# jafarinia/snuffy

Hardware: AMD Instinct MI355X
Metric: slides/sec (higher is better)
Workload: dtype f32; 1 GPU; cfgB: MILNet eval forward, 1 bag/step/rank, N=32768 patches D=768 h=6 Lambda=200 (K=200) depth=1 relu mlp x4; parallelism=bag-parallel x1, bags_resident_per_rank=8, launch=hip graph replay, rccl_ranks=0

## Files before the change

### snuffy_amd/csrc/gemm.hip

```cpp
#include <stdlib.h>

#include "mfma.h"
#include "philox.h"

namespace {

struct GemmParams {
    const unsigned short* a;
    const unsigned short* w;
    const float* bias;
    void* c;
    int64_t lda, ldw, ldc;
    int m, n, k;
    int act;
    int tiles_m, tiles_n;
    unsigned long long* trace;
    const float* resid = nullptr;
    int64_t ldr = 0;
    unsigned int* split_cnt = nullptr;
    float* split_slab = nullptr;
    int split_cap = 0, split_rcap = 0;
    const unsigned short* gate = nullptr;
    int64_t ldg = 0;
    const float* colsum = nullptr;
    const float* rowstats = nullptr;
    unsigned short* c2 = nullptr;
    int64_t ldc2 = 0;
    float* stats_part = nullptr;
    int slots = 0;
    snf::DropoutState drop = {0u, 0u, 0u, 0u, 0u, 1.f};
};
constexpr int HL_SPLIT_MIN_STEPS = 8;
constexpr int HL_SPLIT_MAX = 4;

constexpr int BM = 256, BKS = 32;
constexpr int NBUF = 4, AHEAD = 2;
constexpr int ROWB = BKS * 2;
constexpr int A_BYTES = BM * ROWB;

__device__ __forceinline__ unsigned int cvt_pk_bf16(float lo, float hi) {
    return __builtin_bit_cast(unsigned int, __builtin_convertvector(f32x2{lo, hi}, bf16x2));
}

__device__ __forceinline__ float erf_as(float x) {
    const float ax = fabsf(x);
    const float t = __builtin_amdgcn_rcpf(fmaf(0.3275911f, ax, 1.0f));
    float p = fmaf(1.061405429f, t, -1.453152027f);
    p = fmaf(p, t, 1.421413741f);
    p = fmaf(p, t, -0.284496736f);
    p = fmaf(p, t, 0.254829592f);
    const float e = __builtin_amdgcn_exp2f(-ax * ax * 1.44269504088896340736f);
    return copysignf(fmaf(-p * t, e, 1.0f), x);
}

template <int ACT>
__device__ __forceinline__ float activate(float v) {
    if constexpr (ACT == SNF_ACT_RELU) return fmaxf(v, 0.f);
    if constexpr (ACT == SNF_ACT_GELU) return 0.5f * v * (1.0f + erf_as(v * 0.70710678118654752440f));
    if constexpr (ACT == SNF_ACT_LEAKYRELU) return v > 0.f ? v : 0.01f * v;
    if constexpr (ACT == SNF_ACT_SELU) {
        const float al = 1.6732632423543772848170429916717f, sc = 1.0507009873554804934193349852946f;
        return sc * (v > 0.f ? v : al * (__builtin_amdgcn_exp2f(v * 1.44269504088896340736f) - 1.0f));
    }
    return v;
}

template <int NI, int ACT, int OUT, int EPI = 0, int MI = 8, bool DROP = false>
__global__ __launch_bounds__(512, 2) void gemm_bf16_kernel(GemmParams P) {
    static_assert(!DROP || (ACT == SNF_ACT_RELU && OUT == 0 && EPI == 0), "gemm_bf16: dropout goes with the ReLU -> bf16 form");
    static_assert(MI == 8 || (MI == 4 && NI == 4 && EPI != 1), "gemm_bf16: wave tiles are 128 x 16 NI or 64 x 64");
    constexpr int WC = MI == 8 ? 4 : 2;
    constexpr int RW = 16 * MI;
    static_assert(EPI == 0 || (EPI == 1 ? (NI == 4 && OUT == 0) : ((NI == 4 || NI == 2) && OUT == 1 && ACT == SNF_ACT_NONE)),
                  "gemm_bf16: the LayerNorm-fold epilogue is 256-wide, the residual epilogue 256- or 128-wide");
    constexpr int BN = WC * 16 * NI;
    constexpr int W_BYTES = BN * ROWB;
    constexpr int STEP_BYTES = A_BYTES + W_BYTES;
    constexpr int WP = BN / 128;
    constexpr int GL = 2 + WP;
    constexpr int NC = 4 * NI;
    constexpr bool OUT_F32 = OUT == 1;
    constexpr int NST = EPI == 2 ? NC / 4 + NC / 8 + 1 : (OUT == 1 || OUT == 3) ? NC / 4 : OUT == 2 ? 3 * NC / 8 : NC / 8;
    static_assert((AHEAD - 1) * GL + MI * NST <= 63, "gemm_bf16: counted waits are 6-bit");
    constexpr bool LINE_STORES = OUT == 0 && NI == 4 && EPI != 2 && ACT != SNF_ACT_GELU && ACT != SNF_ACT_SELU;
    extern __shared__ __attribute__((aligned(16))) unsigned char smem[];

// ... 342 lines not shown
        const bool has_next = next < t_hi;
        const Src nxt = tile_src(has_next ? next : tile);
        const bool full = (tile / P.tiles_n + 1) * BM <= P.m && (tile % P.tiles_n + 1) * BN <= P.n;
        for (int s = 0; s < ns; ++s) {
            if constexpr (EPI == 2)
                if (s == 0) preload_x(tile);
            read_frags(rb);
            if (s == ns - 1) load_bias(tile);
            const bool in_tile = s + AHEAD < ns;
            const int exist = has_next ? AHEAD : (ns - 1 - s < AHEAD ? ns - 1 - s : AHEAD);
            if (in_tile)
                stage(cur, s + AHEAD, sb);
            else if (has_next)
                stage(nxt, s + AHEAD - ns, sb);
            if (exist == AHEAD) {
                if (after_epilogue)
                    wait_vmcnt<(AHEAD - 1) * GL + MI * NST>();
                else
                    wait_vmcnt<(AHEAD - 1) * GL>();
            } else if (AHEAD == 3 && exist == 2) {
                wait_vmcnt<GL>();
            } else {
                wait_vmcnt<0>();
            }
            after_epilogue = false;
            rb = rb == NBUF - 1 ? 0 : rb + 1;
            sb = sb == NBUF - 1 ? 0 : sb + 1;
            barrier();
            if (s == 0)
                mma(std::true_type{});
            else
                mma(std::false_type{});
            barrier();
        }
        bias_landed();
#ifdef SNF_GEMM_NOSTORE
        if (false) {
#else
        if (full) {
#endif
            epilogue(tile, std::true_type{});
            after_epilogue = true;
        } else {
            epilogue(tile, std::false_type{});
            wait_vmcnt<0>();
        }
        if (!has_next) break;
        tile = next;
        cur = nxt;
    }
    if (wid < 4) __builtin_amdgcn_s_barrier();
}

template <int ACT, int OUT, bool SPLIT = false, bool GATE = false, bool DROP = false>
__global__ __launch_bounds__(512, 2) void gemm_hl_kernel(GemmParams P) {
    static_assert(!GATE || (OUT == 3 && ACT == SNF_ACT_NONE && !SPLIT), "gemm_hl: the gated form writes an hl image, no activation, no split");
    static_assert(!DROP || (!GATE && (OUT == 1 || OUT == 3)), "gemm_hl: dropout goes with the fp32 and the hl-image outputs");
    constexpr int NI = 4, BN = 256;
    constexpr int ROWL = 128;
    constexpr int IMG = BM * ROWL;
    constexpr int STEP_BYTES = 2 * IMG;
    constexpr int NC = 4 * NI;
    constexpr bool LINE_STORES = (OUT == 1 || OUT == 3) && ACT != SNF_ACT_GELU && ACT != SNF_ACT_SELU;
    extern __shared__ __attribute__((aligned(16))) unsigned char smem[];

    const int lane = threadIdx.x & 63;
    const int wid = __builtin_amdgcn_readfirstlane(threadIdx.x >> 6);
    const int wr = wid >> 2, wc = wid & 3;
    const int ns_all = P.k / BKS;
    unsigned char* const scr = smem + 2 * STEP_BYTES + wid * 4096;

    const int ntiles = P.tiles_m * P.tiles_n;
    const int xcd = blockIdx.x & 7, wg_in_xcd = blockIdx.x >> 3, wgs_per_xcd = gridDim.x >> 3;
    if constexpr (!SPLIT) {
        if (P.split_cap >= 2 && blockIdx.x == 0) {
            for (int i = threadIdx.x; i < 8 * P.split_rcap; i += 512) P.split_cnt[i] = 0u;
            asm volatile("s_waitcnt vmcnt(0)" ::: "memory");
        }
    }
    int t_lo, t_hi;
    {
        const int q = ntiles >> 3, r = ntiles & 7;
        t_lo = xcd < r ? xcd * (q + 1) : r * (q + 1) + (xcd - r) * q;
        t_hi = t_lo + q + (xcd < r ? 1 : 0);
    }
    int sp_part = 0, sp_parts = 1, sp_slot = 0, sp_tile = -1;
    if (P.split_cap >= 2) {
        const int q_x = t_hi - t_lo, full_rounds = q_x / wgs_per_xcd, r = q_x - full_rounds * wgs_per_xcd;
        int sn = r > 0 ? wgs_per_xcd / r : 0;
        if (sn > P.split_cap) sn = P.split_cap;
        if (sn > ns_all / HL_SPLIT_MIN_STEPS) sn = ns_all / HL_SPLIT_MIN_STEPS;
        if (sn >= 2 && r <= P.split_rcap) {
            if constexpr (SPLIT) {
                if (wg_in_xcd < r * sn) {
                    const int jr = wg_in_xcd % r;
                    sp_tile = t_lo + full_rounds * wgs_per_xcd + jr;
                    sp_part = wg_in_xcd / r, sp_parts = sn, sp_slot = xcd * P.split_rcap + jr;
                }
            } else {
                t_hi = t_lo + full_rounds * wgs_per_xcd;
            }
        }
    }
    int tile = t_lo + wg_in_xcd;
    if constexpr (SPLIT) {
        tile = __builtin_amdgcn_readfirstlane(sp_tile);
        sp_part = __builtin_amdgcn_readfirstlane(sp_part), sp_parts = __builtin_amdgcn_readfirstlane(sp_parts);
        sp_slot = __builtin_amdgcn_readfirstlane(sp_slot);
        if (tile < 0) return;
        t_hi = tile + 1;
        asm volatile("" : "+s"(t_hi));
    } else {
        if (tile >= t_hi) return;
    }
    const int s_begin = SPLIT ? __builtin_amdgcn_readfirstlane(sp_part * ns_all / sp_parts) : 0;
    const int ns = SPLIT ? __builtin_amdgcn_readfirstlane((sp_part + 1) * ns_all / sp_parts) - s_begin : ns_all;
    const unsigned short* const a_base = P.a + (SPLIT ? s_begin * 64 : 0);
    const unsigned short* const w_base = P.w + (SPLIT ? s_begin * 64 : 0);

    struct Src {
        int a[4], w[4];
    };
    auto tile_src_mn = [&](int tm, int tn) __attribute__((always_inline)) -> Src {
        Src s;
        int ln = lane;
        asm volatile("" : "+v"(ln));
        const int c = ln & 7;
#pragma unroll
        for (int j = 0; j < 4; ++j) {
            const int row = (4 * wid + j) * 8 + (ln >> 3);
            int grow = tm * BM + row;
            if (grow > P.m - 1) grow = P.m - 1;
            s.a[j] = grow * (int)P.lda + ((c ^ ((row >> 1) & 7)) << 3);
            int wrow = tn * BN + row;
            if (wrow > P.n - 1) wrow = P.n - 1;
            s.w[j] = wrow * (int)P.ldw + ((c ^ (((row >> 1) & 1) | (((row >> 3) & 3) << 1))) << 3);
        }
        return s;
    };
    auto tile_src = [&](int tl) __attribute__((always_inline)) -> Src {
        const int tm = tl / P.tiles_n;
        return tile_src_mn(tm, tl - tm * P.tiles_n);
    };
    auto stage = [&](const Src& s, int kstep, int buf) __attribute__((always_inline)) {
#ifdef X3_NOSTAGE
        return;
#endif
        unsigned char* base = smem + buf * STEP_BYTES;
#pragma unroll
        for (int j = 0; j < 4; ++j) {
            __builtin_amdgcn_global_load_lds((glb_void*)(a_base + s.a[j] + kstep * 64), (lds_void*)(base + (4 * wid + j) * 1024), 16, 0, 0);
            __builtin_amdgcn_global_load_lds((glb_void*)(w_base + s.w[j] + kstep * 64), (lds_void*)(base + IMG + (4 * wid + j) * 1024), 16, 0, 0);
        }
    };

    const int fi = lane & 15, fg = lane >> 4;
    const int fa = (fi >> 1) & 7, fw = ((fi >> 1) & 1) | ((fi >> 2) << 1);
    const int xoff_h = (128 * wr + fi) * ROWL + ((fg ^ fa) << 4), xoff_l = (128 * wr + fi) * ROWL + (((4 + fg) ^ fa) << 4);
    const int wrow0 = IMG + (64 * wc + 8 * (fi >> 2) + (fi & 3)) * ROWL;
    const int woff_h = wrow0 + ((fg ^ fw) << 4), woff_l = wrow0 + (((4 + fg) ^ fw) << 4);

    f32x4 acc[8][NI];
    bf16x8 xf[8], wh[NI], wl[NI];
    f32x4 bv4[NC / 4];

    auto frag = [&](const unsigned char* p) __attribute__((always_inline)) -> bf16x8 {
#ifdef X3_NOREAD
        u32x4 z = {1u, 2u, 3u, (unsigned)lane};
        asm volatile("" : "+v"(z));
        return __builtin_bit_cast(bf16x8, z);
#endif
// ... 81 lines not shown
                    } else if (ok) {
                        *reinterpret_cast<f32x4*>(dst) = f32x4{v[0], v[1], v[2], v[3]};
                        *reinterpret_cast<f32x4*>(dst + 4) = f32x4{v[4], v[5], v[6], v[7]};
                    }
                } else {
                    const u32x4 pk = {cvt_pk_bf16(v[0], v[1]), cvt_pk_bf16(v[2], v[3]), cvt_pk_bf16(v[4], v[5]), cvt_pk_bf16(v[6], v[7])};
                    if constexpr (OUT == 0) {
                        unsigned short* dst = reinterpret_cast<unsigned short*>(P.c) + (int64_t)row * P.ldc + col;
                        if (ok) *reinterpret_cast<u32x4*>(dst) = pk;
                    } else {
                        float lo[8];
#pragma unroll
                        for (int e = 0; e < 8; ++e)
                            lo[e] = v[e] - __uint_as_float((e & 1) ? (pk[e >> 1] & 0xffff0000u) : (pk[e >> 1] << 16));
                        const u32x4 pl = {cvt_pk_bf16(lo[0], lo[1]), cvt_pk_bf16(lo[2], lo[3]), cvt_pk_bf16(lo[4], lo[5]), cvt_pk_bf16(lo[6], lo[7])};
                        unsigned short* dst = reinterpret_cast<unsigned short*>(P.c) + (int64_t)row * P.ldc + 64 * (col >> 5) + (col & 31);
                        if constexpr (LINE_STORES) {
                            *reinterpret_cast<u32x4*>(scr + fio * 256 + (((8 * h + fgo) ^ fio) << 4)) = pk;
                            *reinterpret_cast<u32x4*>(scr + fio * 256 + (((8 * h + 4 + fgo) ^ fio) << 4)) = pl;
                        } else if (ok) {
                            *reinterpret_cast<u32x4*>(dst) = pk;
                            *reinterpret_cast<u32x4*>(dst + 32) = pl;
                        }
                    }
                }
            }
            if constexpr (LINE_STORES) {
                const int lr = lane_o >> 4, lc = lane_o & 15;
                unsigned char* const crow = reinterpret_cast<unsigned char*>(P.c) +
                                            (OUT == 1 ? 4 * (int64_t)(tn * BN + 64 * wc) : 2 * 2 * (int64_t)(tn * BN + 64 * wc));
                const int64_t pitch = (OUT == 1 ? 4 : 2) * P.ldc;
#pragma unroll
                for (int jj = 0; jj < 4; ++jj) {
                    const int r = lr + 4 * jj;
                    const u32x4 val = *reinterpret_cast<const u32x4*>(scr + r * 256 + ((lc ^ r) << 4));
                    const int orow = tm * BM + 128 * wr + 16 * mi + r;
                    const int ocol = tn * BN + 64 * wc + (OUT == 1 ? 4 * lc : 32 * (lc >> 3) + 8 * (lc & 3));
#ifdef X3_NOSTORE
                    const bool ok2 = val[0] == 0x12345678u && orow < 0;
#else
                    const bool ok2 = FULL || (orow < P.m && ocol + (OUT == 1 ? 4 : 8) <= P.n);
#endif
                    if (ok2) *reinterpret_cast<u32x4*>(crow + orow * pitch + 16 * lc) = val;
                }
            }
        }
    };

    Src cur = tile_src(tile);
    stage(cur, 0, 0);
    int buf = 0;
    bool after_epilogue = false;
    while (true) {
        const int next = tile + wgs_per_xcd;
        const bool has_next = next < t_hi;
        const bool full = (tile / P.tiles_n + 1) * BM <= P.m && (tile % P.tiles_n + 1) * BN <= P.n;
        for (int s = 0; s < ns; ++s) {
            if (!(s == 0 && after_epilogue)) wait_vmcnt<0>();
            after_epilogue = false;
            __builtin_amdgcn_sched_barrier(0);
            __builtin_amdgcn_s_barrier();
            __builtin_amdgcn_sched_barrier(0);
            const unsigned char* base = smem + buf * STEP_BYTES;
#pragma unroll
            for (int ni = 0; ni < NI; ++ni) wh[ni] = frag(base + woff_h + (4 * (ni & 1) + 32 * (ni >> 1)) * ROWL);
#pragma unroll
            for (int mi = 0; mi < 8; ++mi) xf[mi] = frag(base + xoff_h + mi * 16 * ROWL);
#pragma unroll
            for (int ni = 0; ni < NI; ++ni) wl[ni] = frag(base + woff_l + (4 * (ni & 1) + 32 * (ni >> 1)) * ROWL);
            __builtin_amdgcn_sched_barrier(0);
            if (s + 1 < ns) {
                stage(cur, s + 1, buf ^ 1);
            } else if (has_next) {
                cur = tile_src(next);
                stage(cur, 0, buf ^ 1);
            }
            __builtin_amdgcn_sched_barrier(0);
            __builtin_amdgcn_s_setprio(1);
            if (s == 0) {
#pragma unroll
                for (int mi = 0; mi < 8; ++mi)
#pragma unroll
                    for (int ni = 0; ni < NI; ++ni) acc[mi][ni] = X3_MFMA(wh[ni], xf[mi], (f32x4{0.f, 0.f, 0.f, 0.f}));
            } else {
#pragma unroll
                for (int mi = 0; mi < 8; ++mi)
#pragma unroll
                    for (int ni = 0; ni < NI; ++ni) acc[mi][ni] = X3_MFMA(wh[ni], xf[mi], acc[mi][ni]);
            }
#pragma unroll
            for (int mi = 0; mi < 8; ++mi) {
#pragma unroll
                for (int ni = 0; ni < NI; ++ni) acc[mi][ni] = X3_MFMA(wl[ni], xf[mi], acc[mi][ni]);
                __builtin_amdgcn_sched_barrier(0);
                xf[mi] = frag(base + xoff_l + mi * 16 * ROWL);
                __builtin_amdgcn_sched_barrier(0);
            }
#pragma unroll
            for (int mi = 0; mi < 8; ++mi)
#pragma unroll
                for (int ni = 0; ni < NI; ++ni) acc[mi][ni] = X3_MFMA(wh[ni], xf[mi], acc[mi][ni]);
            __builtin_amdgcn_s_setprio(0);
            buf ^= 1;
        }
        if constexpr (SPLIT) {
            volatile unsigned int& s_ticket = *reinterpret_cast<volatile unsigned int*>(smem);
            float* slab0 = P.split_slab + (size_t)sp_slot * P.split_cap * (size_t)(BM * BN);
            unsigned tix = threadIdx.x;
            asm volatile("" : "+v"(tix));
            f32x4* mine = reinterpret_cast<f32x4*>(slab0 + (size_t)sp_part * (BM * BN)) + tix;
            wait_vmcnt<0>();
#pragma unroll
            for (int mi = 0; mi < 8; ++mi)
#pragma unroll
                for (int ni = 0; ni < NI; ++ni) mine[(mi * NI + ni) * 512] = acc[mi][ni];
            wait_vmcnt<0>();
            __syncthreads();
            if (tix == 0) {
                __builtin_amdgcn_fence(__ATOMIC_RELEASE, "agent");
                asm volatile("s_waitcnt vmcnt(0)" ::: "memory");
                s_ticket = __hip_atomic_fetch_add(P.split_cnt + sp_slot, 1u, __ATOMIC_RELAXED, __HIP_MEMORY_SCOPE_AGENT);
            }
            __syncthreads();
            if (s_ticket != (unsigned)(sp_parts - 1)) return;
            __syncthreads();
            if (tix == 0) {
                __builtin_amdgcn_fence(__ATOMIC_ACQUIRE, "agent");
                __hip_atomic_store(P.split_cnt + sp_slot, 0u, __ATOMIC_RELAXED, __HIP_MEMORY_SCOPE_AGENT);
            }
            __syncthreads();
#pragma unroll
            for (int mi = 0; mi < 8; ++mi)
#pragma unroll
                for (int ni = 0; ni < NI; ++ni) {
                    f32x4 sum = {0.f, 0.f, 0.f, 0.f};
                    for (int pp = 0; pp < sp_parts; ++pp) {
                        f32x4 v = acc[mi][ni];
                        if (pp != sp_part) v = reinterpret_cast<const f32x4*>(slab0 + (size_t)pp * (BM * BN))[(mi * NI + ni) * 512 + tix];
                        sum = pp == 0 ? v : sum + v;
                    }
                    acc[mi][ni] = sum;
                }
        }
        load_bias(tile);
        wait_vmcnt<0>();
        bias_landed();
        if (full)
            epilogue(tile, std::true_type{});
        else
            epilogue(tile, std::false_type{});
        after_epilogue = true;
        if (!has_next) break;
        tile = next;
    }
}

template <int ACT, int OUT, bool DROP = false>
int launch_hl(const GemmParams& P, hipStream_t s) {
    constexpr int lds = 2 * 2 * BM * 128 + (((OUT == 1 || OUT == 3) && ACT != SNF_ACT_GELU && ACT != SNF_ACT_SELU) ? 8 * 4096 : 0);
    auto kern = [] {
        if constexpr (DROP) return gemm_hl_kernel<ACT, OUT, false, false, true>;
        else return gemm_hl_kernel<ACT, OUT>;
    }();
    static thread_local unsigned long long attr_set_mask = 0;
    if (int rc = snf::lds_opt_in(reinterpret_cast<const void*>(kern), lds, &attr_set_mask, "gemm_hl")) return rc;
    const int ntiles = P.tiles_m * P.tiles_n;
    int grid = snf::cu_count() & ~7;
    if (grid < 8) grid = 8;
    {
        static const int dbg_grid = getenv("SNF_GEMM_HL_GRID") ? atoi(getenv("SNF_GEMM_HL_GRID")) & ~7 : 0;
        if (dbg_grid >= 8 && dbg_grid < grid && P.split_cap < 2) grid = dbg_grid;
    }
    const int per_xcd = (ntiles + 7) / 8;
    if (per_xcd * 8 < grid) grid = per_xcd * 8;
    hipLaunchKernelGGL(kern, dim3(grid), dim3(512), lds, s, P);
    int rc = snf::check_launch("gemm_hl_kernel");
    if (rc || P.split_cap < 2) return rc;
    auto kern2 = [] {
        if constexpr (DROP) return gemm_hl_kernel<ACT, OUT, true, false, true>;
        else return gemm_hl_kernel<ACT, OUT, true>;
    }();
    static thread_local unsigned long long attr_set2_mask = 0;
    if (int rc = snf::lds_opt_in(reinterpret_cast<const void*>(kern2), lds, &attr_set2_mask, "gemm_hl")) return rc;
    hipLaunchKernelGGL(kern2, dim3(grid), dim3(512), lds, s, P);
    return snf::check_launch("gemm_hl_kernel<split>");
}

int launch_hl_gated(const GemmParams& P, hipStream_t s) {
    constexpr int lds = 2 * 2 * BM * 128 + 8 * 4096;
    auto kern = gemm_hl_kernel<SNF_ACT_NONE, 3, false, true>;
    static thread_local unsigned long long attr_set_mask = 0;
    if (int rc = snf::lds_opt_in(reinterpret_cast<const void*>(kern), lds, &attr_set_mask, "gemm_hl")) return rc;
    const int ntiles = P.tiles_m * P.tiles_n;
    int grid = snf::cu_count() & ~7;
    if (grid < 8) grid = 8;
    const int per_xcd = (ntiles + 7) / 8;
    if (per_xcd * 8 < grid) grid = per_xcd * 8;
    hipLaunchKernelGGL(kern, dim3(grid), dim3(512), lds, s, P);
    return snf::check_launch("gemm_hl_kernel<gated>");
}

template <int OUT>
int launch_hl_act(const GemmParams& P, hipStream_t s) {
    switch (P.act) {
        case SNF_ACT_RELU: return launch_hl<SNF_ACT_RELU, OUT>(P, s);
        case SNF_ACT_GELU: return launch_hl<SNF_ACT_GELU, OUT>(P, s);
        case SNF_ACT_LEAKYRELU: return launch_hl<SNF_ACT_LEAKYRELU, OUT>(P, s);
        case SNF_ACT_SELU: return launch_hl<SNF_ACT_SELU, OUT>(P, s);
        default: return launch_hl<SNF_ACT_NONE, OUT>(P, s);
    }
}

template <int NI, int ACT, int OUT, int EPI = 0, int MI = 8, bool DROP = false>
int launch(const GemmParams& P, hipStream_t s) {
    constexpr int lds = NBUF * (A_BYTES + (MI == 8 ? 64 : 32) * NI * ROWB) +
                        ((EPI == 2 || (OUT == 0 && NI == 4 && ACT != SNF_ACT_GELU && ACT != SNF_ACT_SELU)) ? 8 * 4096 : 0);
    auto kern = [] {
        if constexpr (DROP) return gemm_bf16_kernel<NI, ACT, OUT, EPI, MI, true>;
        else return gemm_bf16_kernel<NI, ACT, OUT, EPI, MI>;
    }();
    static thread_local unsigned long long attr_set_mask = 0;
    if (int rc = snf::lds_opt_in(reinterpret_cast<const void*>(kern), lds, &attr_set_mask, "gemm_bf16")) return rc;
    const int ntiles = P.tiles_m * P.tiles_n;
    int grid = snf::cu_count() & ~7;
    if (grid < 8) grid = 8;
    const int per_xcd = (ntiles + 7) / 8;
    if (per_xcd * 8 < grid) grid = per_xcd * 8;
    hipLaunchKernelGGL(kern, dim3(grid), dim3(512), lds, s, P);
    return snf::check_launch("gemm_bf16_kernel");
}

#ifndef SNF_GEMM_128_MI4
#define SNF_GEMM_128_MI4 1
#endif
template <int NI, int ACT, int OUT, int EPI = 0, bool DROP = false>
int launch_tile(const GemmParams& P, hipStream_t s) {
    if constexpr (NI == 2 && SNF_GEMM_128_MI4)
        return launch<4, ACT, OUT, EPI, 4, DROP>(P, s);
// ... 260 lines not shown
    P.c = c;
    P.lda = lda, P.ldw = ldw, P.ldc = ldc;
    P.m = (int)m, P.n = n, P.k = k, P.act = act;
    P.tiles_m = (int)((m + BM - 1) / BM);
    P.tiles_n = (n + 255) / 256;
    P.trace = nullptr;
    return P;
}
}

extern "C" int snf_gemm_bf16_lnfold(const void* a, int64_t lda, const void* w, int64_t ldw, const float* colsum, const float* bias,
                                    const float* rowstats, int64_t m, int n, int k, int act, void* c, int64_t ldc, snf_stream_t stream) {
    SNF_REQUIRE(a && w && c && colsum && bias && rowstats, "snf_gemm_bf16_lnfold: null pointer");
    SNF_REQUIRE(m >= 1 && n >= 1 && k >= 1, "snf_gemm_bf16_lnfold: bad shape m=%lld n=%d k=%d", (long long)m, n, k);
    SNF_REQUIRE(act == SNF_ACT_NONE || act == SNF_ACT_GELU, "snf_gemm_bf16_lnfold: activation %d not built (none, gelu)", act);
    int rc = epi_domain("snf_gemm_bf16_lnfold", a, lda, w, ldw, m, n, k);
    if (rc) return rc;
    SNF_REQUIRE(ldc >= n && ldc % 8 == 0 && reinterpret_cast<uintptr_t>(c) % 16 == 0 && reinterpret_cast<uintptr_t>(colsum) % 16 == 0 &&
                    reinterpret_cast<uintptr_t>(bias) % 16 == 0 && reinterpret_cast<uintptr_t>(rowstats) % 8 == 0,
                "snf_gemm_bf16_lnfold: output / vector alignment");
    GemmParams P = epi_params(a, lda, w, ldw, bias, m, n, k, act, c, ldc);
    P.colsum = colsum, P.rowstats = rowstats;
    hipStream_t s = snf::as_stream(stream);
    return act == SNF_ACT_GELU ? launch<4, SNF_ACT_GELU, 0, 1>(P, s) : launch<4, SNF_ACT_NONE, 0, 1>(P, s);
}

extern "C" int snf_gemm_bf16_resid(const void* a, int64_t lda, const void* w, int64_t ldw, const float* bias, int64_t m, int n, int k,
                                   float* x, int64_t ldx, void* x_bf16, int64_t ldxb, float* stats_part, snf_stream_t stream) {
    SNF_REQUIRE(a && w && x && x_bf16 && stats_part && bias, "snf_gemm_bf16_resid: null pointer");
    SNF_REQUIRE(m >= 1 && n >= 1 && k >= 1, "snf_gemm_bf16_resid: bad shape m=%lld n=%d k=%d", (long long)m, n, k);
    int rc = epi_domain("snf_gemm_bf16_resid", a, lda, w, ldw, m, n, k);
    if (rc) return rc;
    SNF_REQUIRE(ldx >= n && ldx % 4 == 0 && ldxb >= n && ldxb % 8 == 0 && reinterpret_cast<uintptr_t>(x) % 16 == 0 &&
                    reinterpret_cast<uintptr_t>(x_bf16) % 16 == 0 && reinterpret_cast<uintptr_t>(bias) % 16 == 0 &&
                    reinterpret_cast<uintptr_t>(stats_part) % 16 == 0 && m * ldx < 0x7fffffffll,
                "snf_gemm_bf16_resid: output / vector alignment");
    GemmParams P = epi_params(a, lda, w, ldw, bias, m, n, k, SNF_ACT_NONE, x, ldx);
    P.c2 = reinterpret_cast<unsigned short*>(x_bf16), P.ldc2 = ldxb;
    P.stats_part = stats_part, P.slots = n / 32;
    const int rem = n % 256;
    if (rem >= 1 && rem <= 128) {
        P.tiles_n = (n + 127) / 128;
        return launch_tile<2, SNF_ACT_NONE, 1, 2>(P, snf::as_stream(stream));
    }
    return launch<4, SNF_ACT_NONE, 1, 2>(P, snf::as_stream(stream));
}

extern "C" int snf_gemm_hl_bf16(const void* a_hl, int64_t lda, const void* w_hl, int64_t ldw, const float* bias, int64_t m, int n,
                                int k, int act, void* c, int64_t ldc, int out_dtype, snf_stream_t stream) {
    return snf_gemm_hl_resid_bf16(a_hl, lda, w_hl, ldw, bias, nullptr, 0, m, n, k, act, c, ldc, out_dtype, stream);
}

namespace {
struct HlSplit {
    int cap, rcap;
};
HlSplit hl_split_geometry(int64_t m, int n, int k) {
    HlSplit g = {0, 0};
    if (m < 1 || n < 1 || k < BKS) return g;
    const int64_t ntiles64 = ((m + BM - 1) / BM) * ((n + 255) / 256);
    if (ntiles64 > 0x7fffffff) return g;
    const int ntiles = (int)ntiles64, ns = k / BKS;
    int grid = snf::cu_count() & ~7;
    if (grid < 8) grid = 8;
    const int per_xcd = (ntiles + 7) / 8;
    if (per_xcd * 8 < grid) grid = per_xcd * 8;
    const int w = grid >> 3;
    if (ntiles > 2 * grid) return g;
    for (int x = 0; x < 8; ++x) {
        const int q = ntiles / 8 + (x < (ntiles & 7) ? 1 : 0), r = q % w;
        if (r == 0) continue;
        int sn = w / r;
        if (sn > HL_SPLIT_MAX) sn = HL_SPLIT_MAX;
        if (sn > ns / HL_SPLIT_MIN_STEPS) sn = ns / HL_SPLIT_MIN_STEPS;
        if (sn < 2) continue;
        if (sn > g.cap) g.cap = sn;
        if (r > g.rcap) g.rcap = r;
    }
    if (g.cap < 2) g.cap = g.rcap = 0;
    return g;
}
constexpr size_t HL_TICKET_BYTES = 4096;
}

extern "C" size_t snf_gemm_hl_ws_bytes(int64_t m, int n, int k) {
    const HlSplit g = hl_split_geometry(m, n, k);
    if (g.cap < 2 || 8 * g.rcap * sizeof(unsigned int) > HL_TICKET_BYTES) return 0;
    return HL_TICKET_BYTES + (size_t)8 * g.rcap * g.cap * (size_t)(BM * 256) * sizeof(float);
}

extern "C" int snf_gemm_hl_resid_bf16(const void* a_hl, int64_t lda, const void* w_hl, int64_t ldw, const float* bias,
                                      const float* resid, int64_t ldr, int64_t m, int n, int k, int act, void* c, int64_t ldc,
                                      int out_dtype, snf_stream_t stream) {
    return snf_gemm_hl_ws_bf16(a_hl, lda, w_hl, ldw, bias, resid, ldr, m, n, k, act, c, ldc, out_dtype, nullptr, 0, stream);
}

namespace {
int gemm_hl_ws_impl(const void* a_hl, int64_t lda, const void* w_hl, int64_t ldw, const float* bias, const float* resid, int64_t ldr,
                    int64_t m, int n, int k, int act, void* c, int64_t ldc, int out_dtype, const snf::DropoutState* drop, void* workspace,
                    size_t workspace_bytes, snf_stream_t stream) {
    SNF_REQUIRE(a_hl && w_hl && c, "snf_gemm_hl_bf16: null pointer");
    SNF_REQUIRE(m >= 1 && n >= 1 && k >= 1, "snf_gemm_hl_bf16: bad shape m=%lld n=%d k=%d", (long long)m, n, k);
    SNF_REQUIRE(act >= SNF_ACT_RELU && act <= SNF_ACT_NONE, "snf_gemm_hl_bf16: bad activation code %d", act);
    SNF_REQUIRE(out_dtype == SNF_DT_F32 || out_dtype == SNF_DT_BF16 || out_dtype == SNF_DT_BF16_HL,
                "snf_gemm_hl_bf16: bad output dtype %d", out_dtype);
    const bool hl_out = out_dtype == SNF_DT_BF16_HL;
    SNF_REQUIRE(!resid || (out_dtype == SNF_DT_F32 && ldr >= n && ldr % 4 == 0 && reinterpret_cast<uintptr_t>(resid) % 16 == 0),
                "snf_gemm_hl_bf16: a residual needs an fp32 output and 16-byte aligned rows (ldr=%lld)", (long long)ldr);
    if (k % BKS || k < BKS || n % 8 || (hl_out && n % 32) || lda % 8 || ldw % 8 || ldc % (out_dtype == SNF_DT_F32 ? 4 : 8) ||
        lda < 2 * (int64_t)k || ldw < 2 * (int64_t)k || ldc < (hl_out ? 2 * (int64_t)n : n) ||
        (reinterpret_cast<uintptr_t>(a_hl) | reinterpret_cast<uintptr_t>(w_hl) | reinterpret_cast<uintptr_t>(c)) % 16 ||
        (bias && reinterpret_cast<uintptr_t>(bias) % 16) || m * lda >= 0x7fffffffll || (int64_t)n * ldw >= 0x7fffffffll) {
        snf::set_error("snf_gemm_hl_bf16: shape m=%lld n=%d k=%d (lda %lld ldw %lld ldc %lld) outside the kernel's domain "
                       "(k %% 32, n %% 8 (%% 32 for an hl output), images of 2 k columns, 16-byte aligned rows, 31-bit element offsets)",
                       (long long)m, n, k, (long long)lda, (long long)ldw, (long long)ldc);
        return SNF_EUNSUPPORTED;
    }
    GemmParams P;
    P.a = reinterpret_cast<const unsigned short*>(a_hl);
    P.w = reinterpret_cast<const unsigned short*>(w_hl);
    P.bias = bias;
    P.c = c;
    P.lda = lda, P.ldw = ldw, P.ldc = ldc;
    P.m = (int)m, P.n = n, P.k = k, P.act = act;
    P.tiles_m = (int)((m + BM - 1) / BM);
    P.tiles_n = (n + 255) / 256;
    P.trace = nullptr;
    P.resid = resid;
    P.ldr = ldr;
    if (workspace) {
        const size_t need = snf_gemm_hl_ws_bytes(m, n, k);
        if (need) {
            if (workspace_bytes < need || reinterpret_cast<uintptr_t>(workspace) % 16) {
                snf::set_error("snf_gemm_hl_ws_bf16: workspace %zu < %zu (or not 16-byte aligned)", workspace_bytes, need);
                return SNF_EWORKSPACE;
            }
            const HlSplit g = hl_split_geometry(m, n, k);
            P.split_cnt = reinterpret_cast<unsigned int*>(workspace);
            P.split_slab = reinterpret_cast<float*>(reinterpret_cast<unsigned char*>(workspace) + HL_TICKET_BYTES);
            P.split_cap = g.cap, P.split_rcap = g.rcap;
        }
    }
    hipStream_t s = snf::as_stream(stream);
    if (drop && drop->thresh) {
        P.drop = *drop;
        if (hl_out && act == SNF_ACT_RELU && !resid) return launch_hl<SNF_ACT_RELU, 3, true>(P, s);
        if (out_dtype == SNF_DT_F32 && act == SNF_ACT_NONE) return launch_hl<SNF_ACT_NONE, 1, true>(P, s);
        snf::set_error("snf_gemm_hl_dropout_bf16: dropout exists for act = relu with an hl-image output and for act = none with an fp32 "
                       "output (got act %d, out_dtype %d)", act, out_dtype);
        return SNF_EUNSUPPORTED;
    }
    if (hl_out) return launch_hl_act<3>(P, s);
    return out_dtype == SNF_DT_F32 ? launch_hl_act<1>(P, s) : launch_hl_act<0>(P, s);
}
}

extern "C" int snf_gemm_hl_ws_bf16(const void* a_hl, int64_t lda, const void* w_hl, int64_t ldw, const float* bias,
                                   const float* resid, int64_t ldr, int64_t m, int n, int k, int act, void* c, int64_t ldc,
                                   int out_dtype, void* workspace, size_t workspace_bytes, snf_stream_t stream) {
    return gemm_hl_ws_impl(a_hl, lda, w_hl, ldw, bias, resid, ldr, m, n, k, act, c, ldc, out_dtype, nullptr, workspace, workspace_bytes, stream);
}

extern "C" int snf_gemm_hl_ws_dropout_bf16(const void* a_hl, int64_t lda, const void* w_hl, int64_t ldw, const float* bias,
                                           const float* resid, int64_t ldr, int64_t m, int n, int k, int act, void* c, int64_t ldc,
                                           int out_dtype, float dropout_p, uint64_t seed, uint64_t offset, void* workspace,
                                           size_t workspace_bytes, snf_stream_t stream) {
    SNF_REQUIRE(dropout_p >= 0.f && dropout_p < 1.f, "snf_gemm_hl_dropout_bf16: dropout_p=%f outside [0, 1)", dropout_p);
    const snf::DropoutState st = snf::make_dropout(dropout_p, seed, offset);
    return gemm_hl_ws_impl(a_hl, lda, w_hl, ldw, bias, resid, ldr, m, n, k, act, c, ldc, out_dtype, &st, workspace, workspace_bytes, stream);
}

extern "C" int snf_gemm_hl_dropout_bf16(const void* a_hl, int64_t lda, const void* w_hl, int64_t ldw, const float* bias,
                                        const float* resid, int64_t ldr, int64_t m, int n, int k, int act, void* c, int64_t ldc,
                                        int out_dtype, float dropout_p, uint64_t seed, uint64_t offset, snf_stream_t stream) {
    return snf_gemm_hl_ws_dropout_bf16(a_hl, lda, w_hl, ldw, bias, resid, ldr, m, n, k, act, c, ldc, out_dtype, dropout_p, seed, offset,
                                       nullptr, 0, stream);
}

extern "C" int snf_gemm_hl_gated_bf16(const void* a_hl, int64_t lda, const void* w_hl, int64_t ldw, const void* gate_hl, int64_t ldg, int64_t m,
                                      int n, int k, void* c_hl, int64_t ldc, snf_stream_t stream) {
    SNF_REQUIRE(a_hl && w_hl && gate_hl && c_hl, "snf_gemm_hl_gated_bf16: null pointer");
    SNF_REQUIRE(m >= 1 && n >= 1 && k >= 1, "snf_gemm_hl_gated_bf16: bad shape m=%lld n=%d k=%d", (long long)m, n, k);
    if (k % BKS || k < BKS || n % 32 || lda % 8 || ldw % 8 || ldc % 8 || ldg % 8 || lda < 2 * (int64_t)k || ldw < 2 * (int64_t)k ||
        ldc < 2 * (int64_t)n || ldg < 2 * (int64_t)n ||
        (reinterpret_cast<uintptr_t>(a_hl) | reinterpret_cast<uintptr_t>(w_hl) | reinterpret_cast<uintptr_t>(c_hl) |
         reinterpret_cast<uintptr_t>(gate_hl)) % 16 ||
        m * lda >= 0x7fffffffll || (int64_t)n * ldw >= 0x7fffffffll) {
        snf::set_error("snf_gemm_hl_gated_bf16: shape m=%lld n=%d k=%d (lda %lld ldw %lld ldc %lld ldg %lld) outside the kernel's domain "
                       "(k %% 32, n %% 32, images of 2 k / 2 n columns, 16-byte aligned rows, 31-bit element offsets)",
                       (long long)m, n, k, (long long)lda, (long long)ldw, (long long)ldc, (long long)ldg);
        return SNF_EUNSUPPORTED;
    }
    GemmParams P;
// ... 47 lines not shown
```

Measured before the change: 905.7 slides/s.

## Replace two-launch tail split-K with single balanced stream-K walk over tile units

```diff
diff --git a/snuffy_amd/csrc/gemm.hip b/snuffy_amd/csrc/gemm.hip
--- a/snuffy_amd/csrc/gemm.hip
+++ b/snuffy_amd/csrc/gemm.hip
@@ -1,5 +1,6 @@
 #include <stdlib.h>
 
+#include "hl_walk.h"
 #include "mfma.h"
 #include "philox.h"
 
@@ -19,7 +20,6 @@
     int64_t ldr = 0;
     unsigned int* split_cnt = nullptr;
     float* split_slab = nullptr;
-    int split_cap = 0, split_rcap = 0;
     const unsigned short* gate = nullptr;
     int64_t ldg = 0;
     const float* colsum = nullptr;
@@ -30,8 +30,9 @@
     int slots = 0;
     snf::DropoutState drop = {0u, 0u, 0u, 0u, 0u, 1.f};
 };
-constexpr int HL_SPLIT_MIN_STEPS = 8;
-constexpr int HL_SPLIT_MAX = 4;
+using snf_hl_walk::HL_SPLIT_MAX;
+using snf_hl_walk::HL_SPLIT_MIN_STEPS;
+constexpr size_t HL_TICKET_BYTES = 8 * snf_hl_walk::HL_MAX_WGS_PER_XCD * sizeof(unsigned int);
 
 constexpr int BM = 256, BKS = 32;
 constexpr int NBUF = 4, AHEAD = 2;
@@ -480,9 +481,9 @@
     if (wid < 4) __builtin_amdgcn_s_barrier();
 }
 
-template <int ACT, int OUT, bool SPLIT = false, bool GATE = false, bool DROP = false>
+template <int ACT, int OUT, bool BAL = false, bool GATE = false, bool DROP = false>
 __global__ __launch_bounds__(512, 2) void gemm_hl_kernel(GemmParams P) {
-    static_assert(!GATE || (OUT == 3 && ACT == SNF_ACT_NONE && !SPLIT), "gemm_hl: the gated form writes an hl image, no activation, no split");
+    static_assert(!GATE || (OUT == 3 && ACT == SNF_ACT_NONE && !BAL), "gemm_hl: the gated form writes an hl image, no activation, no split");
     static_assert(!DROP || (!GATE && (OUT == 1 || OUT == 3)), "gemm_hl: dropout goes with the fp32 and the hl-image outputs");
     constexpr int NI = 4, BN = 256;
     constexpr int ROWL = 128;
@@ -500,51 +501,29 @@
 
     const int ntiles = P.tiles_m * P.tiles_n;
     const int xcd = blockIdx.x & 7, wg_in_xcd = blockIdx.x >> 3, wgs_per_xcd = gridDim.x >> 3;
-    if constexpr (!SPLIT) {
-        if (P.split_cap >= 2 && blockIdx.x == 0) {
-            for (int i = threadIdx.x; i < 8 * P.split_rcap; i += 512) P.split_cnt[i] = 0u;
-            asm volatile("s_waitcnt vmcnt(0)" ::: "memory");
-        }
-    }
     int t_lo, t_hi;
     {
         const int q = ntiles >> 3, r = ntiles & 7;
         t_lo = xcd < r ? xcd * (q + 1) : r * (q + 1) + (xcd - r) * q;
         t_hi = t_lo + q + (xcd < r ? 1 : 0);
     }
-    int sp_part = 0, sp_parts = 1, sp_slot = 0, sp_tile = -1;
-    if (P.split_cap >= 2) {
-        const int q_x = t_hi - t_lo, full_rounds = q_x / wgs_per_xcd, r = q_x - full_rounds * wgs_per_xcd;
-        int sn = r > 0 ? wgs_per_xcd / r : 0;
-        if (sn > P.split_cap) sn = P.split_cap;
-        if (sn > ns_all / HL_SPLIT_MIN_STEPS) sn = ns_all / HL_SPLIT_MIN_STEPS;
-        if (sn >= 2 && r <= P.split_rcap) {
-            if constexpr (SPLIT) {
-                if (wg_in_xcd < r * sn) {
-                    const int jr = wg_in_xcd % r;
-                    sp_tile = t_lo + full_rounds * wgs_per_xcd + jr;
-                    sp_part = wg_in_xcd / r, sp_parts = sn, sp_slot = xcd * P.split_rcap + jr;
-                }
-            } else {
-                t_hi = t_lo + full_rounds * wgs_per_xcd;
-            }
-        }
-    }
     int tile = t_lo + wg_in_xcd;
-    if constexpr (SPLIT) {
-        tile = __builtin_amdgcn_readfirstlane(sp_tile);
-        sp_part = __builtin_amdgcn_readfirstlane(sp_part), sp_parts = __builtin_amdgcn_readfirstlane(sp_parts);
-        sp_slot = __builtin_amdgcn_readfirstlane(sp_slot);
-        if (tile < 0) return;
-        t_hi = tile + 1;
-        asm volatile("" : "+s"(t_hi));
+    int ns = ns_all;
+    const unsigned short* a_base = P.a;
+    const unsigned short* w_base = P.w;
+    int rem = 0;
+    if constexpr (BAL) {
+        const int units = snf_hl_walk::units_per_tile(ns_all), bal_n = (t_hi - t_lo) * units;
+        const int bal_w = wgs_per_xcd < bal_n ? wgs_per_xcd : bal_n;
+        if (wg_in_xcd >= bal_w) return;
+        const snf_hl_walk::Walk wk = snf_hl_walk::walk_begin(wg_in_xcd, ns_all, bal_n, bal_w);
+        tile = t_lo + __builtin_amdgcn_readfirstlane(wk.tile);
+        ns = __builtin_amdgcn_readfirstlane(wk.ns), rem = __builtin_amdgcn_readfirstlane(wk.rem);
+        const int s_begin = __builtin_amdgcn_readfirstlane(wk.s_begin);
+        a_base += s_begin * 64, w_base += s_begin * 64;
     } else {
         if (tile >= t_hi) return;
     }
-    const int s_begin = SPLIT ? __builtin_amdgcn_readfirstlane(sp_part * ns_all / sp_parts) : 0;
-    const int ns = SPLIT ? __builtin_amdgcn_readfirstlane((sp_part + 1) * ns_all / sp_parts) - s_begin : ns_all;
-    const unsigned short* const a_base = P.a + (SPLIT ? s_begin * 64 : 0);
-    const unsigned short* const w_base = P.w + (SPLIT ? s_begin * 64 : 0);
 
     struct Src {
         int a[4], w[4];
@@ -732,8 +711,8 @@
     int buf = 0;
     bool after_epilogue = false;
     while (true) {
-        const int next = tile + wgs_per_xcd;
-        const bool has_next = next < t_hi;
+        const int next = BAL ? tile + 1 : tile + wgs_per_xcd;
+        const bool has_next = BAL ? rem > 0 : next < t_hi;
         const bool full = (tile / P.tiles_n + 1) * BM <= P.m && (tile % P.tiles_n + 1) * BN <= P.n;
         for (int s = 0; s < ns; ++s) {
             if (!(s == 0 && after_epilogue)) wait_vmcnt<0>();
@@ -753,6 +732,7 @@
                 stage(cur, s + 1, buf ^ 1);
             } else if (has_next) {
                 cur = tile_src(next);
+                if constexpr (BAL) a_base = P.a, w_base = P.w;
                 stage(cur, 0, buf ^ 1);
             }
             __builtin_amdgcn_sched_barrier(0);
@@ -783,45 +763,54 @@
             __builtin_amdgcn_s_setprio(0);
             buf ^= 1;
         }
-        if constexpr (SPLIT) {
-            volatile unsigned int& s_ticket = *reinterpret_cast<volatile unsigned int*>(smem);
-            float* slab0 = P.split_slab + (size_t)sp_slot * P.split_cap * (size_t)(BM * BN);
-            unsigned tix = threadIdx.x;
-            asm volatile("" : "+v"(tix));
-            f32x4* mine = reinterpret_cast<f32x4*>(slab0 + (size_t)sp_part * (BM * BN)) + tix;
-            wait_vmcnt<0>();
-#pragma unroll
-            for (int mi = 0; mi < 8; ++mi)
-#pragma unroll
-                for (int ni = 0; ni < NI; ++ni) mine[(mi * NI + ni) * 512] = acc[mi][ni];
-            wait_vmcnt<0>();
-            __syncthreads();
-            if (tix == 0) {
-                __builtin_amdgcn_fence(__ATOMIC_RELEASE, "agent");
-                asm volatile("s_waitcnt vmcnt(0)" ::: "memory");
-                s_ticket = __hip_atomic_fetch_add(P.split_cnt + sp_slot, 1u, __ATOMIC_RELAXED, __HIP_MEMORY_SCOPE_AGENT);
-            }
-            __syncthreads();
-            if (s_ticket != (unsigned)(sp_parts - 1)) return;
-            __syncthreads();
-            if (tix == 0) {
-                __builtin_amdgcn_fence(__ATOMIC_ACQUIRE, "agent");
-                __hip_atomic_store(P.split_cnt + sp_slot, 0u, __ATOMIC_RELAXED, __HIP_MEMORY_SCOPE_AGENT);
-            }
-            __syncthreads();
-#pragma unroll
-            for (int mi = 0; mi < 8; ++mi)
-#pragma unroll
-                for (int ni = 0; ni < NI; ++ni) {
-                    f32x4 sum = {0.f, 0.f, 0.f, 0.f};
-                    for (int pp = 0; pp < sp_parts; ++pp) {
-                        f32x4 v = acc[mi][ni];
-                        if (pp != sp_part) v = reinterpret_cast<const f32x4*>(slab0 + (size_t)pp * (BM * BN))[(mi * NI + ni) * 512 + tix];
-                        sum = pp == 0 ? v : sum + v;
-                    }
-                    acc[mi][ni] = sum;
+        bool parked = false;
+        if constexpr (BAL) {
+            if (ns != ns_all) {
+                volatile unsigned int& s_ticket = *reinterpret_cast<volatile unsigned int*>(smem + (buf ^ 1) * STEP_BYTES);
+                const int bal_n = (t_hi - t_lo) * snf_hl_walk::units_per_tile(ns_all), bal_w = wgs_per_xcd < bal_n ? wgs_per_xcd : bal_n;
+                const snf_hl_walk::Parts tp = snf_hl_walk::tile_parts(tile - t_lo, ns_all, bal_n, bal_w);
+                const int wg0 = __builtin_amdgcn_readfirstlane(tp.wg0), sp_parts = __builtin_amdgcn_readfirstlane(tp.parts);
+                const int sp_part = wg_in_xcd - wg0;
+                unsigned int* const ticket = P.split_cnt + snf_hl_walk::ticket_index(xcd, wgs_per_xcd, wg0);
+                unsigned tix = threadIdx.x;
+                asm volatile("" : "+v"(tix));
+                f32x4* mine = reinterpret_cast<f32x4*>(P.split_slab + (size_t)snf_hl_walk::slab_index(xcd, wgs_per_xcd, wg_in_xcd, sp_part) * (size_t)(BM * BN)) + tix;
+                wait_vmcnt<0>();
+#pragma unroll
+                for (int mi = 0; mi < 8; ++mi)
+#pragma unroll
+                    for (int ni = 0; ni < NI; ++ni) mine[(mi * NI + ni) * 512] = acc[mi][ni];
+                wait_vmcnt<0>();
+                __syncthreads();
+                if (tix == 0) {
+                    __builtin_amdgcn_fence(__ATOMIC_RELEASE, "agent");
+                    asm volatile("s_waitcnt vmcnt(0)" ::: "memory");
+                    s_ticket = __hip_atomic_fetch_add(ticket, 1u, __ATOMIC_RELAXED, __HIP_MEMORY_SCOPE_AGENT);
                 }
-        }
+                __syncthreads();
+                parked = s_ticket != (unsigned)(sp_parts - 1);
+                if (!parked) {
+                    __syncthreads();
+                    if (tix == 0) __builtin_amdgcn_fence(__ATOMIC_ACQUIRE, "agent");
+                    __syncthreads();
+#pragma unroll
+                    for (int mi = 0; mi < 8; ++mi)
+#pragma unroll
+                        for (int ni = 0; ni < NI; ++ni) {
+                            f32x4 sum = {0.f, 0.f, 0.f, 0.f};
+                            for (int pp = 0; pp < sp_parts; ++pp) {
+                                f32x4 v = acc[mi][ni];
+                                if (pp != sp_part)
+                                    v = reinterpret_cast<const f32x4*>(P.split_slab + (size_t)snf_hl_walk::slab_index(xcd, wgs_per_xcd, wg0 + pp, pp) *
+                                                                                          (size_t)(BM * BN))[(mi * NI + ni) * 512 + tix];
+                                sum = pp == 0 ? v : sum + v;
+                            }
+                            acc[mi][ni] = sum;
+                        }
+                }
+            }
+        }
+        if (!parked) {
         load_bias(tile);
         wait_vmcnt<0>();
         bias_landed();
@@ -830,40 +819,54 @@
         else
             epilogue(tile, std::false_type{});
         after_epilogue = true;
+        }
         if (!has_next) break;
         tile = next;
-    }
+        if constexpr (BAL) {
+            snf_hl_walk::Walk wk = {0, 0, ns, rem};
+            snf_hl_walk::walk_next(wk, ns_all);
+            ns = __builtin_amdgcn_readfirstlane(wk.ns), rem = wk.rem;
+        }
+    }
+}
+
+int hl_walk_wgs(int ntiles, int ns) {
+    int grid = snf::cu_count() & ~7;
+    if (grid < 8) grid = 8;
+    return snf_hl_walk::launch_wgs(ntiles, ns, grid >> 3);
 }
 
 template <int ACT, int OUT, bool DROP = false>
 int launch_hl(const GemmParams& P, hipStream_t s) {
     constexpr int lds = 2 * 2 * BM * 128 + (((OUT == 1 || OUT == 3) && ACT != SNF_ACT_GELU && ACT != SNF_ACT_SELU) ? 8 * 4096 : 0);
+    const int ntiles = P.tiles_m * P.tiles_n;
+    if (P.split_cnt) {
+        auto kern = [] {
+            if constexpr (DROP) return gemm_hl_kernel<ACT, OUT, true, false, true>;
+            else return gemm_hl_kernel<ACT, OUT, true>;
+        }();
+        static thread_local unsigned long long attr_set_mask = 0;
+        if (int rc = snf::lds_opt_in(reinterpret_cast<const void*>(kern), lds, &attr_set_mask, "gemm_hl")) return rc;
+        if (hipMemsetAsync(P.split_cnt, 0, HL_TICKET_BYTES, s) != hipSuccess) return snf::check_launch("gemm_hl_kernel<balanced> tickets");
+        hipLaunchKernelGGL(kern, dim3(8 * hl_walk_wgs(ntiles, P.k / BKS)), dim3(512), lds, s, P);
+        return snf::check_launch("gemm_hl_kernel<balanced>");
+    }
     auto kern = [] {
         if constexpr (DROP) return gemm_hl_kernel<ACT, OUT, false, false, true>;
         else return gemm_hl_kernel<ACT, OUT>;
     }();
     static thread_local unsigned long long attr_set_mask = 0;
     if (int rc = snf::lds_opt_in(reinterpret_cast<const void*>(kern), lds, &attr_set_mask, "gemm_hl")) return rc;
-    const int ntiles = P.tiles_m * P.tiles_n;
     int grid = snf::cu_count() & ~7;
     if (grid < 8) grid = 8;
     {
         static const int dbg_grid = getenv("SNF_GEMM_HL_GRID") ? atoi(getenv("SNF_GEMM_HL_GRID")) & ~7 : 0;
-        if (dbg_grid >= 8 && dbg_grid < grid && P.split_cap < 2) grid = dbg_grid;
+        if (dbg_grid >= 8 && dbg_grid < grid) grid = dbg_grid;
     }
     const int per_xcd = (ntiles + 7) / 8;
     if (per_xcd * 8 < grid) grid = per_xcd * 8;
     hipLaunchKernelGGL(kern, dim3(grid), dim3(512), lds, s, P);
-    int rc = snf::check_launch("gemm_hl_kernel");
-    if (rc || P.split_cap < 2) return rc;
-    auto kern2 = [] {
-        if constexpr (DROP) return gemm_hl_kernel<ACT, OUT, true, false, true>;
-        else return gemm_hl_kernel<ACT, OUT, true>;
-    }();
-    static thread_local unsigned long long attr_set2_mask = 0;
-    if (int rc = snf::lds_opt_in(reinterpret_cast<const void*>(kern2), lds, &attr_set2_mask, "gemm_hl")) return rc;
-    hipLaunchKernelGGL(kern2, dim3(grid), dim3(512), lds, s, P);
-    return snf::check_launch("gemm_hl_kernel<split>");
+    return snf::check_launch("gemm_hl_kernel");
 }
 
 int launch_hl_gated(const GemmParams& P, hipStream_t s) {
@@ -1230,21 +1233,18 @@
 }
 
 namespace {
-struct HlSplit {
-    int cap, rcap;
-};
-HlSplit hl_split_geometry(int64_t m, int n, int k) {
-    HlSplit g = {0, 0};
-    if (m < 1 || n < 1 || k < BKS) return g;
+bool hl_walk_domain(int64_t m, int n, int k) {
+    if (m < 1 || n < 1 || k < BKS) return false;
     const int64_t ntiles64 = ((m + BM - 1) / BM) * ((n + 255) / 256);
-    if (ntiles64 > 0x7fffffff) return g;
+    if (ntiles64 > 0x7fffffff) return false;
     const int ntiles = (int)ntiles64, ns = k / BKS;
     int grid = snf::cu_count() & ~7;
     if (grid < 8) grid = 8;
     const int per_xcd = (ntiles + 7) / 8;
     if (per_xcd * 8 < grid) grid = per_xcd * 8;
     const int w = grid >> 3;
-    if (ntiles > 2 * grid) return g;
+    if (ntiles > 2 * grid) return false;
+    int cap = 0, rcap = 0;
     for (int x = 0; x < 8; ++x) {
         const int q = ntiles / 8 + (x < (ntiles & 7) ? 1 : 0), r = q % w;
         if (r == 0) continue;
@@ -1252,19 +1252,17 @@
         if (sn > HL_SPLIT_MAX) sn = HL_SPLIT_MAX;
         if (sn > ns / HL_SPLIT_MIN_STEPS) sn = ns / HL_SPLIT_MIN_STEPS;
         if (sn < 2) continue;
-        if (sn > g.cap) g.cap = sn;
-        if (r > g.rcap) g.rcap = r;
-    }
-    if (g.cap < 2) g.cap = g.rcap = 0;
-    return g;
-}
-constexpr size_t HL_TICKET_BYTES = 4096;
+        if (sn > cap) cap = sn;
+        if (r > rcap) rcap = r;
+    }
+    return cap >= 2 && 8 * rcap * sizeof(unsigned int) <= 4096;
+}
 }
 
 extern "C" size_t snf_gemm_hl_ws_bytes(int64_t m, int n, int k) {
-    const HlSplit g = hl_split_geometry(m, n, k);
-    if (g.cap < 2 || 8 * g.rcap * sizeof(unsigned int) > HL_TICKET_BYTES) return 0;
-    return HL_TICKET_BYTES + (size_t)8 * g.rcap * g.cap * (size_t)(BM * 256) * sizeof(float);
+    if (!hl_walk_domain(m, n, k)) return 0;
+    const int ntiles = (int)(((m + BM - 1) / BM) * ((n + 255) / 256));
+    return HL_TICKET_BYTES + (size_t)8 * snf_hl_walk::slabs_per_xcd(hl_walk_wgs(ntiles, k / BKS)) * (size_t)(BM * 256) * sizeof(float);
 }
 
 extern "C" int snf_gemm_hl_resid_bf16(const void* a_hl, int64_t lda, const void* w_hl, int64_t ldw, const float* bias,
@@ -1313,10 +1311,8 @@
                 snf::set_error("snf_gemm_hl_ws_bf16: workspace %zu < %zu (or not 16-byte aligned)", workspace_bytes, need);
                 return SNF_EWORKSPACE;
             }
-            const HlSplit g = hl_split_geometry(m, n, k);
             P.split_cnt = reinterpret_cast<unsigned int*>(workspace);
             P.split_slab = reinterpret_cast<float*>(reinterpret_cast<unsigned char*>(workspace) + HL_TICKET_BYTES);
-            P.split_cap = g.cap, P.split_rcap = g.rcap;
         }
     }
     hipStream_t s = snf::as_stream(stream);
diff --git a/snuffy_amd/csrc/hl_walk.h b/snuffy_amd/csrc/hl_walk.h
--- /dev/null
+++ b/snuffy_amd/csrc/hl_walk.h
@@ -0,0 +1,77 @@
+#pragma once
+
+#if defined(__HIPCC__) || defined(__CUDACC__)
+#define SNF_HL_WALK_FN __host__ __device__ inline
+#else
+#define SNF_HL_WALK_FN inline
+#endif
+
+namespace snf_hl_walk {
+
+constexpr int HL_SPLIT_MIN_STEPS = 8;
+constexpr int HL_SPLIT_MAX = 4;
+constexpr int HL_MAX_WGS_PER_XCD = 128;
+
+SNF_HL_WALK_FN int units_per_tile(int ns) {
+    int u = ns / HL_SPLIT_MIN_STEPS;
+    if (u > HL_SPLIT_MAX) u = HL_SPLIT_MAX;
+    return u < 1 ? 1 : u;
+}
+SNF_HL_WALK_FN int unit_step(int j, int ns, int units) { return j * ns / units; }
+
+SNF_HL_WALK_FN int xcd_tiles(int ntiles, int x, int* t_lo) {
+    const int q = ntiles >> 3, r = ntiles & 7;
+    *t_lo = x < r ? x * (q + 1) : r * (q + 1) + (x - r) * q;
+    return q + (x < r ? 1 : 0);
+}
+
+SNF_HL_WALK_FN int launch_wgs(int ntiles, int ns, int wgs_cap) {
+    const int n_max = ((ntiles + 7) >> 3) * units_per_tile(ns);
+    int w = wgs_cap < n_max ? wgs_cap : n_max;
+    if (w > HL_MAX_WGS_PER_XCD) w = HL_MAX_WGS_PER_XCD;
+    return w < 1 ? 1 : w;
+}
+SNF_HL_WALK_FN int xcd_wgs(int tiles_x, int ns, int wgs) {
+    const int n = tiles_x * units_per_tile(ns);
+    return wgs < n ? wgs : n;
+}
+SNF_HL_WALK_FN int wg_cut(int i, int n, int w) { return (int)((long long)i * n / w); }
+SNF_HL_WALK_FN int unit_owner(int u, int n, int w) { return (int)((((long long)u + 1) * w - 1) / n); }
+
+SNF_HL_WALK_FN int slabs_per_xcd(int wgs) { return 2 * wgs; }
+SNF_HL_WALK_FN int slab_index(int x, int wgs, int wg, int part) { return x * slabs_per_xcd(wgs) + 2 * wg + (part == 0 ? 1 : 0); }
+SNF_HL_WALK_FN int ticket_index(int x, int wgs, int wg0) { return x * wgs + wg0; }
+
+struct Walk {
+    int tile, s_begin, ns, rem;
+};
+SNF_HL_WALK_FN Walk walk_begin(int wg, int ns_all, int n, int w) {
+    const int units = units_per_tile(ns_all);
+    const int u = wg_cut(wg, n, w), u_hi = wg_cut(wg + 1, n, w);
+    Walk k;
+    k.tile = u / units;
+    const int o = u - k.tile * units, o_end = u_hi - k.tile * units < units ? u_hi - k.tile * units : units;
+    k.s_begin = unit_step(o, ns_all, units);
+    k.ns = unit_step(o_end, ns_all, units) - k.s_begin;
+    k.rem = u_hi - k.tile * units - o_end;
+    return k;
+}
+SNF_HL_WALK_FN void walk_next(Walk& k, int ns_all) {
+    const int units = units_per_tile(ns_all), o_end = k.rem < units ? k.rem : units;
+    k.tile += 1;
+    k.s_begin = 0;
+    k.ns = unit_step(o_end, ns_all, units);
+    k.rem -= o_end;
+}
+struct Parts {
+    int wg0, parts;
+};
+SNF_HL_WALK_FN Parts tile_parts(int tile, int ns_all, int n, int w) {
+    const int units = units_per_tile(ns_all);
+    Parts p;
+    p.wg0 = unit_owner(tile * units, n, w);
+    p.parts = unit_owner(tile * units + units - 1, n, w) - p.wg0 + 1;
+    return p;
+}
+
+}
```

After: 888.9 slides/s. -1.9%, worse.
